# pyannote/pyannote-audio

Measured on AMD Instinct MI355X. Metric: audio-hours/sec (real-time factor) for speaker-diarization-3.1 pipeline, higher is better.
Workload: dtype f32

## Files before the change

pyannote-audio_amd/csrc/emb_winograd4.hip:

```cpp
#include <stdlib.h>

#include <type_traits>

#include "common.h"
#include "emb_winograd_geom.h"
#include "emb_winograd4_geom.h"

namespace pa {

typedef float f32x2 __attribute__((ext_vector_type(2)));
typedef __attribute__((address_space(3))) void* lds4_ptr_t;

typedef const volatile f32x2 __attribute__((address_space(3))) * w4_lds_f32x2_ptr;
__device__ __forceinline__ f32x2 w4_lds_read64(const unsigned char* p) { return *(w4_lds_f32x2_ptr)p; }

__device__ __forceinline__ void wino4_barrier() {
  asm volatile("s_waitcnt lgkmcnt(0)" ::: "memory");
  __builtin_amdgcn_s_barrier();
  asm volatile("" ::: "memory");
}

struct W4Const {
  f32x2 p4, m4, m5, p2, m2, m1;
};
__device__ __forceinline__ f32x2 w4fma(f32x2 a, f32x2 b, f32x2 c) { return __builtin_elementwise_fma(a, b, c); }
__device__ __forceinline__ void wino4_bt(const f32x2 (&x)[6], f32x2 (&y)[6], const W4Const& k) {
  const f32x2 a = w4fma(x[2], k.m4, x[4]);
  const f32x2 b = w4fma(x[1], k.m4, x[3]);
  const f32x2 c = w4fma(x[2], k.m1, x[4]);
  const f32x2 d = w4fma(x[1], k.m1, x[3]);
  y[0] = w4fma(x[0], k.p4, w4fma(x[2], k.m5, x[4]));
  y[1] = a + b;
  y[2] = w4fma(b, k.m1, a);
  y[3] = w4fma(d, k.p2, c);
  y[4] = w4fma(d, k.m2, c);
  y[5] = w4fma(x[1], k.p4, w4fma(x[3], k.m5, x[5]));
}

struct W4Const4 {
  f32x4 m1, p2, p4, p8, m2, m8;
};
__device__ __forceinline__ f32x4 w4fma4(f32x4 a, f32x4 b, f32x4 c) { return __builtin_elementwise_fma(a, b, c); }
__device__ __forceinline__ void wino4_at(const f32x4 m0, const f32x4 m1, const f32x4 m2, const f32x4 m3,
                                         const f32x4 m4, const f32x4 m5, f32x4 (&y)[4], const W4Const4& k) {
  const f32x4 s1 = m1 + m2, d1 = w4fma4(m2, k.m1, m1), s2 = m3 + m4, d2 = w4fma4(m4, k.m1, m3);
  y[0] = m0 + s1 + s2;
  y[1] = w4fma4(d2, k.p2, d1);
  y[2] = w4fma4(s2, k.p4, s1);
  y[3] = w4fma4(d2, k.p8, d1) + m5;
}

#define W4_MFMA_A(acc, a, b) asm volatile("v_mfma_f32_16x16x4_f32 %0, %1, %2, %0" : "+a"(acc) : "v"(a), "v"(b))
#define W4_MFMA_A_ZERO(acc, a, b) asm volatile("v_mfma_f32_16x16x4_f32 %0, %1, %2, 0" : "=a"(acc) : "v"(a), "v"(b))
#define W4_MFMA_V(acc, a, b) asm volatile("v_mfma_f32_16x16x4_f32 %0, %1, %2, %0" : "+v"(acc) : "v"(a), "v"(b))
#define W4_MFMA_V_ZERO(acc, a, b) asm volatile("v_mfma_f32_16x16x4_f32 %0, %1, %2, 0" : "=v"(acc) : "v"(a), "v"(b))

__device__ __forceinline__ float w4_opaque(float v) {
  asm volatile("" : "+s"(v));
  return v;
}

struct Wino4Stage {
  __amdgpu_buffer_rsrc_t xsrd, usrd;
  int keep, usoff;
  unsigned char* pbuf;
  unsigned char* ubuf;
};
struct Wino4Ctx {
  const float* xp;
  int xnum;
  int keep, usoff;
};
__device__ __forceinline__ Wino4Ctx wino4_ctx(const float* __restrict__ X, int H, int W, int CIN, const Wino4Unit& u,
                                              int n0, int x0_last) {
  using G = Wino4Geom;
  const long img = (long)H * W * CIN;
  const long org = ((long)(u.y0 - 1) * W + (u.x0 - 1)) * CIN;
  Wino4Ctx c;
  c.xp = X + (long)u.b * img + org;
  c.xnum = (int)((img - org) * 4);
  c.keep = wino4_patch_keep(u, x0_last);
  c.usoff = (n0 / W_BN) * (CIN / G::CB) * G::USLAB_BYTES;
  return c;
}
__device__ __forceinline__ Wino4Stage wino4_stage(const Wino4Ctx& c, const float* __restrict__ U, int COUT, int CIN,
                                                  int s, unsigned char* pbuf, unsigned char* ubuf) {
  using G = Wino4Geom;
  Wino4Stage st;
  st.xsrd = __builtin_amdgcn_make_buffer_rsrc(const_cast<float*>(c.xp + s * G::CB), 0, c.xnum - s * G::CB * 4,
                                              0x00020000);
  st.usrd = __builtin_amdgcn_make_buffer_rsrc(const_cast<float*>(U), 0, 36 * COUT * CIN * 4, 0x00020000);
  st.keep = c.keep;
  st.usoff = c.usoff + s * G::USLAB_BYTES;
  st.pbuf = pbuf;
  st.ubuf = ubuf;
  return st;
}

#ifndef PA_W4_STAMP
#define PA_W4_STAMP 0
#endif
#ifndef PA_W4_DEFER_STORES
#define PA_W4_DEFER_STORES 1
#endif
#ifndef PA_W4_STORE_AUX
#define PA_W4_STORE_AUX 2
#endif
#ifndef PA_W4_RES_AUX
#define PA_W4_RES_AUX 0
#endif
#ifndef PA_W4_STORES_IN_FLIGHT
#define PA_W4_STORES_IN_FLIGHT 1
#endif
#ifndef PA_W4_LATE_BARRIER
#define PA_W4_LATE_BARRIER 1
#endif
#if PA_W4_STAMP
__device__ unsigned long long g_w4_stamps[8 * 4 * 64 * 10];
#define W4_STAMP(p) st_[p] = __builtin_amdgcn_s_memtime()
#define W4_STAMP_FLUSH()                                                                      \
  do {                                                                                        \
    if (blockIdx.x < 8 && st_iter < 64 && lane == 0) {                                         \
      _Pragma("unroll") for (int p_ = 0; p_ < 10; ++p_)                                        \
          g_w4_stamps[((blockIdx.x * 4 + slw) * 64 + st_iter) * 10 + p_] = st_[p_];            \
    }                                                                                         \
    ++st_iter;                                                                                \
  } while (0)
#else
#define W4_STAMP(p)
#define W4_STAMP_FLUSH()
#endif

constexpr int W4_AGPR_POINTS = 32;
constexpr int W4_U_PIECES = Wino4Geom::UINSTR / 4;
static_assert(W4_U_PIECES == 9 && Wino4Geom::UINSTR % 4 == 0, "36 U pieces of 1 KB per stage, 4 waves");
constexpr int W4_TILE_OUT = 16;
constexpr int W4_TAIL_WAIT = 2 * W4_TILE_OUT;
#define W4_STR2(x) #x
#define W4_STR(x) W4_STR2(x)
#define W4_U_PIECES_LIT 9
#define W4_TAIL_WAIT_LIT 32
static_assert(W4_U_PIECES == W4_U_PIECES_LIT && W4_TAIL_WAIT == W4_TAIL_WAIT_LIT, "the literals of the s_waitcnt strings");

template <int PIN>
struct Wino4Lanes {
  int a[PIN];
};
template <int PIN>
__device__ __forceinline__ void wino4_piece(const int I, const Wino4Stage& st, const Wino4Lanes<PIN>& pl, int lane,
                                            int slw) {
  if (I < PIN) {
    const int off = pl.a[I < PIN ? I : 0] & st.keep;
    __builtin_amdgcn_raw_ptr_buffer_load_lds(st.xsrd, (lds4_ptr_t)(st.pbuf + 1024 * I), 16, off, 0, 0, 0);
  } else {
    const int k = slw + 4 * (I - PIN);
    __builtin_amdgcn_raw_ptr_buffer_load_lds(st.usrd, (lds4_ptr_t)(st.ubuf + 1024 * k), 16, lane * 16,
                                             st.usoff + 1024 * k, 0, 0);
  }
}
struct Wino4Dma {
  unsigned patch_lds;
  unsigned u_lds;
  int usoff;
};
__device__ __forceinline__ unsigned w4_lds_addr(const void* p) {
  return (unsigned)(size_t)(lds4_ptr_t)const_cast<void*>(p);
}
template <int I, int PIN>
__device__ __forceinline__ void wino4_piece_asm(const Wino4Stage& st, const Wino4Dma& d, const int (&plm)[PIN],
                                                int lane16) {
  if constexpr (I < PIN) {
    asm volatile("s_add_u32 m0, %0, %1\n\ts_nop 0\n\tbuffer_load_dwordx4 %2, %3, 0 offen lds"
                 :: "s"(d.patch_lds), "i"(1024 * I), "v"(plm[I]), "s"(st.xsrd)
                 : "memory");
  } else {
    int tmp;
    asm volatile("s_add_u32 m0, %1, %2\n\ts_add_u32 %0, %3, %2\n\tbuffer_load_dwordx4 %4, %5, %0 offen lds"
                 : "=&s"(tmp)
                 : "s"(d.u_lds), "i"(4096 * (I - PIN)), "s"(d.usoff), "v"(lane16), "s"(st.usrd)
                 : "memory");
  }
}
template <int PIN>
__device__ __forceinline__ void wino4_piece_asm_n(const int piece, const Wino4Stage& st, const Wino4Dma& d,
                                                  const int (&plm)[PIN], int lane16) {
  switch (piece) {
#define W4_CASE(I) case I: if constexpr (I < PIN + W4_U_PIECES) wino4_piece_asm<I, PIN>(st, d, plm, lane16); break;
    W4_CASE(0) W4_CASE(1) W4_CASE(2) W4_CASE(3) W4_CASE(4) W4_CASE(5) W4_CASE(6) W4_CASE(7) W4_CASE(8) W4_CASE(9)
    W4_CASE(10) W4_CASE(11) W4_CASE(12) W4_CASE(13) W4_CASE(14) W4_CASE(15) W4_CASE(16) W4_CASE(17) W4_CASE(18)
    W4_CASE(19) W4_CASE(20) W4_CASE(21) W4_CASE(22) W4_CASE(23) W4_CASE(24) W4_CASE(25) W4_CASE(26)
#undef W4_CASE
    default: break;
  }
}
template <int PIN>
__device__ __forceinline__ void wino4_issue_all(const Wino4Stage& st, const Wino4Lanes<PIN>& pl, int lane, int slw) {
#pragma unroll
  for (int i = 0; i < PIN + W4_U_PIECES; ++i) wino4_piece<PIN>(i, st, pl, lane, slw);
}

struct Wino4LinUnit {
  int b0;
  Wino4LinTile tc;
};
__device__ __forceinline__ Wino4LinUnit wino4_lin_unit(int u, int tcols, int trows, int total_tiles, int H, int W,
                                                       int CIN, int lane, int (&off)[Wino4LinGeom::PINSTR]) {
  Wino4LinUnit o;
  o.b0 = __builtin_amdgcn_readfirstlane(wino4_lin_b0(u, tcols, trows, total_tiles));
  o.tc = wino4_lin_tile(16 * u + (lane & 15), tcols, trows, total_tiles, o.b0);
  const Wino4LinTile td = wino4_lin_tile(16 * u + ((lane >> 1) & 15), tcols, trows, total_tiles, o.b0);
#pragma unroll
  for (int i = 0; i < Wino4LinGeom::PINSTR; ++i) off[i] = wino4_lin_patch_lane(i, td, H, W, CIN, lane);
  return o;
}
__device__ __forceinline__ Wino4LinUnit wino4_run_unit(int u, int tcols, int trows, int total_tiles, int H, int W,
                                                       int CIN, int nimg, int lane, int (&off)[Wino4RunGeom::PINSTR],
                                                       int* slot) {
  Wino4LinUnit o;
  int b0;
  const Wino4Runs R = wino4_runs(u, tcols, trows, &b0);
  o.b0 = __builtin_amdgcn_readfirstlane(b0);
  const int t = lane & 15;
  o.tc = wino4_run_tile(R, t, u, total_tiles);
  *slot = t + wino4_run_of_tile(R, t);
  wino4_run_patch_lanes(off, R, H, W, CIN, nimg - o.b0, lane);
  return o;
}
__device__ __forceinline__ Wino4Ctx wino4_lin_ctx(const float* __restrict__ X, int H, int W, int CIN, int nimg, int b0,
                                                  int n0) {
  using G = Wino4LinGeom;
  const long img = (long)H * W * CIN;
  const long long rest = (long long)(nimg - b0) * img * 4;
  Wino4Ctx c;
  c.xp = X + (long)b0 * img;
  c.xnum = (int)(rest > 0x7fffffffLL ? 0x7fffffffLL : rest);
  c.keep = -1;
  c.usoff = (n0 / W_BN) * (CIN / G::CB) * G::USLAB_BYTES;
  return c;
}

template <bool HAS_R, int MODE>
__global__ __launch_bounds__(256, 1) void k_conv3x3_wino4(
    const float* __restrict__ X, int H, int W, int CIN, const float* __restrict__ U,
    const float* __restrict__ shift, const float* __restrict__ R, float* __restrict__ Y, int COUT, int relu,
    int cgroups, int trows, int num_units, int num_groups, int n_tiles, int total_work, int nimg, int xranges,
    int* __restrict__ counters) {
  constexpr bool LATE = PA_W4_LATE_BARRIER && MODE == 0;
  constexpr bool LIN = MODE != 0;
  constexpr bool RUN = MODE == 2;
  using G = std::conditional_t<MODE == 0, Wino4Geom, std::conditional_t<MODE == 1, Wino4LinGeom, Wino4RunGeom>>;
  constexpr int PIN = G::PINSTR;
  constexpr int W4_PIECES = PIN + W4_U_PIECES;
  static_assert(W4_PIECES <= 27, "wino4_piece_asm_n spells out 27 cases");
  static_assert(2 * W4_TILE_OUT * (HAS_R ? 2 : 1) >= W4_TAIL_WAIT, "a tile's first-stage wait counts epilogue operations");
  extern __shared__ __attribute__((aligned(16))) unsigned char smem4[];
  const int tid = threadIdx.x, lane = tid & 63;
  const int t = lane & 15, g = lane >> 4;
  const int slw = __builtin_amdgcn_readfirstlane(tid >> 6);
  unsigned char* my_patch = smem4 + slw * G::PATCH_BYTES;
  unsigned char* ubufs = smem4 + 4 * G::PATCH_BYTES;
  int* mail = reinterpret_cast<int*>(smem4 + G::LDS_BYTES);

  const TileQueue tq{counters, (int)(blockIdx.x & 7), total_work >> 3};
  if (tid == 0) mail[0] = tq_resolve(tq, tq_claim_own(tq));
  __syncthreads();
  int q = mail[0];
  if (q < 0) {
    if (tid == 0) tq_done(tq, gridDim.x);
    return;
  }
  const int x0_last = LIN ? 0 : (cgroups - 1) * Wino4Geom::TW;
  Wino4Lanes<PIN> pl;
  Wino4Lanes<PIN> npl;
  if constexpr (!LIN) wino4_patch_lanes(pl.a, W, CIN, lane, x0_last);
#define W4_PATCH_K(i, j) (MODE == 1 ? wino4_lin_patch_k(i, j) : (MODE == 2 ? wino4_run_patch_k(i, j) : wino4_patch_k(i, j)))
  int pbase0 = MODE == 1 ? wino4_lin_patch_base(t, g) : wino4_patch_base(t, g, 0);
  int pbase1 = MODE == 1 ? pbase0 : wino4_patch_base(t, g, 1);
  int nxt_slot = 0;
  const int last_unit = LIN ? ((num_units + 15) >> 4) - 1 : 0;
  const int ubase = wino4_u_base(t, g);
  const int lane16 = lane * 16;
  W4Const kc;
  {
    const float p4 = w4_opaque(4.f), m4 = w4_opaque(-4.f), m5 = w4_opaque(-5.f), p2 = w4_opaque(2.f),
                m2 = w4_opaque(-2.f), m1 = w4_opaque(-1.f);
    kc.p4 = f32x2{p4, p4}; kc.m4 = f32x2{m4, m4}; kc.m5 = f32x2{m5, m5};
    kc.p2 = f32x2{p2, p2}; kc.m2 = f32x2{m2, m2}; kc.m1 = f32x2{m1, m1};
  }
  const int nstages = CIN / G::CB;

  Wino4Work wk = wino4_decode(q, n_tiles, num_groups, xranges);
  Wino4Unit cur = Wino4Unit{0, 0, 0, 0}, nxt = cur;
  Wino4LinUnit lcur = Wino4LinUnit{0, Wino4LinTile{0, 0, 0, 0}}, lnxt = lcur;
  int cur_n0 = wk.n0, nxt_n0 = wk.n0;
  Wino4Ctx cctx;
  if constexpr (RUN) {
    const int uu = wk.unit0 + slw;
    int slot;
    lcur = wino4_run_unit(uu < last_unit ? uu : last_unit, cgroups, trows, num_units, H, W, CIN, nimg, lane, pl.a, &slot);
    lcur.tc.valid &= wk.valid & (uu <= last_unit);
    pbase0 = wino4_run_patch_base(slot, g, 0);
    pbase1 = wino4_run_patch_base(slot, g, 1);
    cctx = wino4_lin_ctx(X, H, W, CIN, nimg, lcur.b0, cur_n0);
  } else if constexpr (LIN) {
    lcur = wino4_lin_unit(wk.unit0 + slw, cgroups, trows, num_units, H, W, CIN, lane, pl.a);
    lcur.tc.valid &= wk.valid;
    cctx = wino4_lin_ctx(X, H, W, CIN, nimg, lcur.b0, cur_n0);
  } else {
    cur = wino4_unit(wk.unit0 + slw, cgroups, trows, num_units);
    cur.valid &= wk.valid;
    cctx = wino4_ctx(X, H, W, CIN, cur, cur_n0, x0_last);
  }
  nxt = cur;
  lnxt = lcur;
  Wino4Ctx nctx = cctx;
  int buf = 0;
  wino4_issue_all<PIN>(wino4_stage(cctx, U, COUT, CIN, 0, my_patch, ubufs), pl, lane, slw);
  int claim = 0;
  if (tid == 0) claim = tq_claim_own(tq);
  int nq = -1;
  bool first_tile = true;
  f32x4 acca[W4_AGPR_POINTS][2];
  f32x4 accv[36 - W4_AGPR_POINTS][2];

#if PA_W4_STAMP
  unsigned long long st_[10] = {0, 0, 0, 0, 0, 0, 0, 0, 0, 0};
  int st_iter = 0;
#endif
  while (true) {
    for (int s = 0; s < nstages; ++s) {
      W4_STAMP(0);
      if constexpr (LATE) {
      if (s == 0) {
        if (PA_W4_STORES_IN_FLIGHT && !first_tile) asm volatile("s_waitcnt vmcnt(" W4_STR(W4_TAIL_WAIT_LIT) ")" ::: "memory");
        else asm volatile("s_waitcnt vmcnt(0)" ::: "memory");
      } else {
        asm volatile("s_waitcnt vmcnt(" W4_STR(W4_U_PIECES_LIT) ")" ::: "memory");
      }
      } else {
        asm volatile("s_waitcnt vmcnt(0)" ::: "memory");
      }
      W4_STAMP(1);
      if (s == nstages - 1 && tid == 0) mail[0] = tq_resolve(tq, claim);
      f32x2 x_first[6];
      asm volatile("s_waitcnt lgkmcnt(0)" ::: "memory");
#pragma unroll
      for (int i = 0; i < 6; ++i)
        x_first[i] = w4_lds_read64(my_patch + pbase0 + W4_PATCH_K(i, 0));
      unsigned char* umine = ubufs + buf * G::USLAB_BYTES;
      unsigned char* uother = ubufs + (buf ^ 1) * G::USLAB_BYTES;
      bool stage_next = true;
      Wino4Stage nst;
      auto stage_barrier = [&]() {
        if constexpr (LATE) asm volatile("s_waitcnt vmcnt(0)" ::: "memory");
        __builtin_amdgcn_s_barrier();
        asm volatile("" ::: "memory");
        W4_STAMP(2);
        if (s + 1 < nstages) {
          nst = wino4_stage(cctx, U, COUT, CIN, s + 1, my_patch, uother);
        } else {
          nq = mail[0];
          stage_next = nq >= 0;
          wk = wino4_decode(stage_next ? nq : 0, n_tiles, num_groups, xranges);
          nxt_n0 = wk.n0;
          if constexpr (LIN) {
            const int uu = wk.unit0 + slw;
            if constexpr (RUN) {
              lnxt = wino4_run_unit(uu < last_unit ? uu : last_unit, cgroups, trows, num_units, H, W, CIN, nimg, lane,
                                    npl.a, &nxt_slot);
              lnxt.tc.valid &= wk.valid & (uu <= last_unit);
            } else {
              lnxt = wino4_lin_unit(uu, cgroups, trows, num_units, H, W, CIN, lane, npl.a);
              lnxt.tc.valid &= wk.valid;
            }
            nctx = wino4_lin_ctx(X, H, W, CIN, nimg, lnxt.b0, nxt_n0);
          } else {
            nxt = wino4_unit(wk.unit0 + slw, cgroups, trows, num_units);
            nxt.valid &= wk.valid;
            nctx = wino4_ctx(X, H, W, CIN, nxt, nxt_n0, x0_last);
          }
          nst = wino4_stage(nctx, U, COUT, CIN, 0, my_patch, uother);
        }
      };
      if constexpr (!LATE) stage_barrier();
      f32x2 v[6][6];
      f32x2 uf_first[2][2];
      {
        const unsigned char* pb0 = my_patch + pbase0;
        const unsigned char* pb1 = my_patch + pbase1;
        f32x2 tt[6][6];
        f32x2 x[2][6];
#define W4_RD(i, j) w4_lds_read64(((j) >> 2 ? pb1 : pb0) + W4_PATCH_K(i, j))
#pragma unroll
        for (int i = 0; i < 6; ++i) x[0][i] = x_first[i];
#pragma unroll
        for (int j = 0; j < 6; ++j) {
          if (j + 1 < 6) {
#pragma unroll
            for (int i = 0; i < 6; ++i) x[(j + 1) & 1][i] = W4_RD(i, j + 1);
          }
          __builtin_amdgcn_sched_barrier(0);
          f32x2 y[6];
          wino4_bt(x[j & 1], y, kc);
#pragma unroll
          for (int i = 0; i < 6; ++i) tt[i][j] = y[i];
          __builtin_amdgcn_sched_barrier(0);
        }
#pragma unroll
        for (int i = 0; i < 6; ++i) {
          if (i == 5) {
            if constexpr (LATE) {
              stage_barrier();
              __builtin_amdgcn_sched_barrier(0);
            }
#pragma unroll
            for (int e = 0; e < 2; ++e)
#pragma unroll
              for (int cg = 0; cg < 2; ++cg) uf_first[e][cg] = w4_lds_read64(umine + ubase + wino4_u_k(e, cg));
            __builtin_amdgcn_sched_barrier(0);
          }
          wino4_bt(tt[i], v[i], kc);
          __builtin_amdgcn_sched_barrier(0);
        }
      }
#if PA_W4_STAMP
      asm volatile("s_nop 0" ::"v"(v[5][5]), "v"(v[0][0]));
#endif
      W4_STAMP(3);
      int plm[PIN];
      if constexpr (LIN) {
#pragma unroll
        for (int i = 0; i < PIN; ++i) plm[i] = s + 1 < nstages ? pl.a[i] : npl.a[i];
      } else {
#pragma unroll
        for (int i = 0; i < PIN; ++i) plm[i] = pl.a[i] & nst.keep;
      }
      const Wino4Dma dma{w4_lds_addr(my_patch), w4_lds_addr(uother) + 1024u * slw, nst.usoff + 1024 * slw};
      auto mfma_run = [&](auto first_stage) {
        constexpr bool FIRST = decltype(first_stage)::value;
        const unsigned char* ub = umine + ubase;
        f32x2 uf[2][2][2];
#pragma unroll
        for (int e = 0; e < 2; ++e)
#pragma unroll
          for (int cg = 0; cg < 2; ++cg) {
            uf[0][e][cg] = uf_first[e][cg];
          }
        __builtin_amdgcn_sched_barrier(0);
#pragma unroll
        for (int xp = 0; xp < 36; xp += 2) {
          const int par = (xp >> 1) & 1;
#pragma unroll
          for (int m = 0; m < 8; ++m) {
            const int ks = m >> 2, e = (m >> 1) & 1, cg = m & 1;
            const int xi = xp + e;
            const f32x2 bv = v[xi / 6][xi % 6];
            const float a = ks ? uf[par][e][cg].y : uf[par][e][cg].x, b = ks ? bv.y : bv.x;
            if (xi < W4_AGPR_POINTS) {
              if (ks == 0 && FIRST) W4_MFMA_A_ZERO(acca[xi < W4_AGPR_POINTS ? xi : 0][cg], a, b);
              else W4_MFMA_A(acca[xi < W4_AGPR_POINTS ? xi : 0][cg], a, b);
            } else {
              if (ks == 0 && FIRST) W4_MFMA_V_ZERO(accv[xi >= W4_AGPR_POINTS ? xi - W4_AGPR_POINTS : 0][cg], a, b);
              else W4_MFMA_V(accv[xi >= W4_AGPR_POINTS ? xi - W4_AGPR_POINTS : 0][cg], a, b);
            }
            __builtin_amdgcn_sched_barrier(0);
            if ((m == 0 || m == 2) && xp + 2 < 36) {
              const int en = m >> 1;
#pragma unroll
              for (int c2 = 0; c2 < 2; ++c2)
                uf[par ^ 1][en][c2] = w4_lds_read64(ub + wino4_u_k(xp + 2 + en, c2));
              __builtin_amdgcn_sched_barrier(0);
            }
            if ((m == 4 || m == 6) && stage_next) {
              const int piece = xp + ((m - 4) >> 1);
              if (piece < W4_PIECES) wino4_piece_asm_n<PIN>(piece, nst, dma, plm, lane16);
              __builtin_amdgcn_sched_barrier(0);
            }
          }
        }
      };
      if (s == 0) mfma_run(std::true_type{});
      else mfma_run(std::false_type{});
      W4_STAMP(4);
      buf ^= 1;
      if (s + 1 < nstages) {
        W4_STAMP(5);
        W4_STAMP_FLUSH();
      }
    }
    if (tid == 0 && nq >= 0) claim = tq_claim_own(tq);
    first_tile = false;
    asm volatile("s_nop 15\n\ts_nop 15" ::: "memory");
    {
      W4Const4 k4;
      {
        const float m1 = w4_opaque(-1.f), p2 = w4_opaque(2.f), p4 = w4_opaque(4.f), p8 = w4_opaque(8.f),
                    m2 = w4_opaque(-2.f), m8 = w4_opaque(-8.f);
        k4.m1 = f32x4{m1, m1, m1, m1}; k4.p2 = f32x4{p2, p2, p2, p2};
        k4.p4 = f32x4{p4, p4, p4, p4}; k4.p8 = f32x4{p8, p8, p8, p8};
        k4.m2 = f32x4{m2, m2, m2, m2}; k4.m8 = f32x4{m8, m8, m8, m8};
      }
      const long oimg = (long)H * W * COUT;
      const int ob = LIN ? lcur.b0 : cur.b;
      const long long orest = (long long)(LIN ? nimg - ob : 1) * oimg * 4;
      const int onum = (int)(orest > 0x7fffffffLL ? 0x7fffffffLL : orest);
      const __amdgpu_buffer_rsrc_t ysrd = __builtin_amdgcn_make_buffer_rsrc(Y + (long)ob * oimg, 0, onum, 0x00020000);
      const __amdgpu_buffer_rsrc_t rsrd = __builtin_amdgcn_make_buffer_rsrc(
          const_cast<float*>(HAS_R ? R + (long)ob * oimg : Y), 0, onum, 0x00020000);
      constexpr int OOB = (int)0x80000000;
      const int xl = LIN ? lcur.tc.x : cur.x0 + 4 * t;
      const int yl = LIN ? lcur.tc.b * H + lcur.tc.y : cur.y0;
      const int rows_ok = LIN ? H - lcur.tc.y : 4;
      const int tile_ok = LIN ? lcur.tc.valid : cur.valid;
      const int obase = ((yl * W + xl) * COUT + cur_n0 + 4 * g) * 4;
      const int srow = W * COUT * 4, spix = COUT * 4;
      int offq[4];
#pragma unroll
      for (int qq = 0; qq < 4; ++qq) offq[qq] = (tile_ok && xl + qq < W) ? obase + qq * spix : OOB;
      auto ooff = [&](const int p, const int qq, const int cg) {
        if constexpr (LIN) return (offq[qq] == OOB || p >= rows_ok) ? OOB : offq[qq] + p * srow + 64 * cg;
        else return offq[qq] == OOB ? OOB : offq[qq] + p * srow + 64 * cg;
      };
      const float lo = relu ? 0.f : -__builtin_inff();
      const f32x4 lo4 = {lo, lo, lo, lo};
#define W4_ACC(xi) ((xi) < W4_AGPR_POINTS ? acca[(xi) < W4_AGPR_POINTS ? (xi) : 0][cg] \
                                          : accv[(xi) >= W4_AGPR_POINTS ? (xi)-W4_AGPR_POINTS : 0][cg])
      constexpr bool DEFER = PA_W4_DEFER_STORES == 2 || (PA_W4_DEFER_STORES == 1 && !HAS_R);
      f32x4 held[4][4];
      auto store_held = [&](const int k) {
        __builtin_amdgcn_raw_buffer_store_b128(__builtin_bit_cast(u32x4, held[k >> 2][k & 3]), ysrd,
                                               ooff(k >> 2, k & 3, 0), 0, PA_W4_STORE_AUX);
      };
#pragma unroll
      for (int cg = 0; cg < 2; ++cg) {
        f32x4 sh;
        {
          const float* sp = shift + cur_n0 + 16 * cg;
          float s16[16];
#pragma unroll
          for (int i = 0; i < 16; ++i) s16[i] = sp[i];
#pragma unroll
          for (int r = 0; r < 4; ++r)
            sh[r] = g == 0 ? s16[r] : (g == 1 ? s16[4 + r] : (g == 2 ? s16[8 + r] : s16[12 + r]));
        }
        f32x4 rv[4][4];
        if (HAS_R) {
#pragma unroll
          for (int p = 0; p < 2; ++p)
#pragma unroll
            for (int qq = 0; qq < 4; ++qq)
              rv[p][qq] = __builtin_bit_cast(
                  f32x4, __builtin_amdgcn_raw_buffer_load_b128(rsrd, ooff(p, qq, cg), 0, PA_W4_RES_AUX));
        }
        __builtin_amdgcn_sched_barrier(0);
        f32x4 o[4][4];
#pragma unroll
        for (int b = 0; b < 6; ++b) {
#pragma unroll
          for (int a6 = 0; a6 < 6; ++a6) {
            const int xi = 6 * a6 + b;
            if (xi < W4_AGPR_POINTS) asm volatile("" : "+a"(acca[xi < W4_AGPR_POINTS ? xi : 0][cg]));
          }
          f32x4 y[4];
          wino4_at(W4_ACC(0 + b), W4_ACC(6 + b), W4_ACC(12 + b), W4_ACC(18 + b), W4_ACC(24 + b), W4_ACC(30 + b), y,
                   k4);
#pragma unroll
          for (int p = 0; p < 4; ++p) {
            if (b == 0) {
              o[p][0] = y[p];
            } else if (b == 1) {
              o[p][0] = o[p][0] + y[p];
              o[p][1] = y[p];
              o[p][2] = y[p];
              o[p][3] = y[p];
            } else if (b == 2) {
              o[p][0] = o[p][0] + y[p];
              o[p][1] = w4fma4(y[p], k4.m1, o[p][1]);
              o[p][2] = o[p][2] + y[p];
              o[p][3] = w4fma4(y[p], k4.m1, o[p][3]);
            } else if (b == 3) {
              o[p][0] = o[p][0] + y[p];
              o[p][1] = w4fma4(y[p], k4.p2, o[p][1]);
              o[p][2] = w4fma4(y[p], k4.p4, o[p][2]);
              o[p][3] = w4fma4(y[p], k4.p8, o[p][3]);
            } else if (b == 4) {
              o[p][0] = o[p][0] + y[p];
              o[p][1] = w4fma4(y[p], k4.m2, o[p][1]);
              o[p][2] = w4fma4(y[p], k4.p4, o[p][2]);
              o[p][3] = w4fma4(y[p], k4.m8, o[p][3]);
            } else {
              o[p][3] = o[p][3] + y[p];
            }
          }
          if (b & 1) __builtin_amdgcn_sched_barrier(0);
          if (DEFER && cg == 1) {
            constexpr int first[7] = {0, 3, 6, 9, 12, 14, 16};
            __builtin_amdgcn_sched_barrier(0);
#pragma unroll
            for (int k = first[b]; k < first[b + 1]; ++k) store_held(k);
            __builtin_amdgcn_sched_barrier(0);
          }
          if (HAS_R && b == 3) {
#pragma unroll
            for (int p = 2; p < 4; ++p)
#pragma unroll
              for (int qq = 0; qq < 4; ++qq)
                rv[p][qq] = __builtin_bit_cast(
                    f32x4, __builtin_amdgcn_raw_buffer_load_b128(rsrd, ooff(p, qq, cg), 0, PA_W4_RES_AUX));
            __builtin_amdgcn_sched_barrier(0);
          }
        }
#if PA_W4_STAMP
        asm volatile("s_nop 0" ::"v"(o[3][3]), "v"(o[0][0]));
        st_[6 + 2 * cg] = __builtin_amdgcn_s_memtime();
#endif
#pragma unroll
        for (int p = 0; p < 4; ++p)
#pragma unroll
          for (int qq = 0; qq < 4; ++qq) {
            o[p][qq] = o[p][qq] + sh;
            if (HAS_R) o[p][qq] = o[p][qq] + rv[p][qq];
            o[p][qq] = __builtin_elementwise_max(o[p][qq], lo4);
          }
        __builtin_amdgcn_sched_barrier(0);
        if (DEFER && cg == 0) {
#pragma unroll
          for (int p = 0; p < 4; ++p)
#pragma unroll
            for (int qq = 0; qq < 4; ++qq) held[p][qq] = o[p][qq];
        } else {
#pragma unroll
          for (int p = 0; p < 4; ++p)
#pragma unroll
            for (int qq = 0; qq < 4; ++qq)
              __builtin_amdgcn_raw_buffer_store_b128(__builtin_bit_cast(u32x4, o[p][qq]), ysrd, ooff(p, qq, cg), 0,
                                                     PA_W4_STORE_AUX);
        }
        __builtin_amdgcn_sched_barrier(0);
#if PA_W4_STAMP
        st_[7 + 2 * cg] = __builtin_amdgcn_s_memtime();
#endif
      }
#undef W4_ACC
    }
    W4_STAMP(5);
    W4_STAMP_FLUSH();
    if (nq < 0) break;
    cur = nxt;
    if constexpr (LIN) {
      lcur = lnxt;
      pl = npl;
      if constexpr (RUN) {
        pbase0 = wino4_run_patch_base(nxt_slot, g, 0);
        pbase1 = wino4_run_patch_base(nxt_slot, g, 1);
      }
    }
    cur_n0 = nxt_n0;
    cctx = nctx;
  }
  if (tid == 0) tq_done(tq, gridDim.x);
}

static int wino4_unit_mode(int B, int H, int W, int rows) {
  if (rows != H) return 0;
  const long tcols = cdiv(W, 4), trows = cdiv(H, 4);
  static const char* e = getenv("PA_WINO4_LINEAR");
  if (e != nullptr) {
    const int m = atoi(e);
    return m == 2 && tcols < 5 ? 1 : m;
  }
  const long lin_units = cdiv((long)B * trows * tcols, 16), row_units = (long)B * trows * cdiv(W, 64);
  if (tcols >= 5 && lin_units * 118 <= row_units * 100) return 2;
  return lin_units * 120 <= row_units * 100 ? 1 : 0;
}

int xcd_ranges_wanted(bool by_default) {
  static const char* e = getenv("PA_XCD_RANGES");
  return e != nullptr ? (atoi(e) != 0) : (by_default ? 1 : 0);
}

template <bool HAS_R, int MODE>
static int launch_wino4(const float* X, int B, int H, int W, int CIN, const float* U, const float* shift,
                        const float* R, float* Y, int COUT, int relu, int rows, hipStream_t st) {
  constexpr bool LIN = MODE != 0;
  using G = std::conditional_t<MODE == 0, Wino4Geom, std::conditional_t<MODE == 1, Wino4LinGeom, Wino4RunGeom>>;
  const int cgroups = LIN ? cdiv(W, 4) : cdiv(W, Wino4Geom::TW), trows = cdiv(rows, 4);
  const size_t lds = (size_t)G::LDS_BYTES + 16;
  auto kernel = k_conv3x3_wino4<HAS_R, MODE>;
  constexpr int MAXDEV = 16;
  static int cus_of[MAXDEV] = {0};
  int dev = 0;
  (void)hipGetDevice(&dev);
  if (dev < 0 || dev >= MAXDEV) dev = 0;
  if (!cus_of[dev]) {
    (void)hipFuncSetAttribute((const void*)kernel, hipFuncAttributeMaxDynamicSharedMemorySize, (int)lds);
    int cus = 256;
    (void)hipDeviceGetAttribute(&cus, hipDeviceAttributeMultiprocessorCount, dev);
    cus_of[dev] = cus;
  }
  const int n_tiles = COUT / W_BN;
  const long total_tiles = (long)cgroups * trows * B;
  const long num_units = LIN ? (total_tiles + 15) / 16 : (long)cgroups * trows * B;
  const long num_groups = (num_units + 3) / 4;
  const long total = ((num_groups + 7) / 8) * 8 * n_tiles;
  const int resident = cus_of[dev] & ~7;
  const int grid = (int)(total < resident ? total : resident);
  int* counters = tile_counters();
  if (counters == nullptr) {
    set_error("pa_conv3x3_wino4: cannot allocate the tile counters");
    return 2;
  }
  hipLaunchKernelGGL(kernel, dim3(grid), dim3(256), lds, st, X, H, W, CIN, U, shift, R, Y, COUT, relu, cgroups, trows,
                     (int)(LIN ? total_tiles : num_units), (int)num_groups, n_tiles, (int)total, B,
                     xcd_ranges_wanted(n_tiles < 8), counters);
  return 0;
}

}

extern "C" {

#if PA_W4_STAMP
int pa_wino4_read_stamps(unsigned long long* host) {
  (void)hipDeviceSynchronize();
  return hipMemcpyFromSymbol(host, HIP_SYMBOL(pa::g_w4_stamps), sizeof(unsigned long long) * 8 * 4 * 64 * 10) ==
                 hipSuccess
             ? 0
             : 1;
}
#endif

int pa_conv3x3_wino4_rows(const float* X, int B, int H, int W, int cin, const float* U, const float* shift,
                          const float* R, float* Y, int cout, int relu, int rows, void* stream);

int pa_conv3x3_wino4(const float* X, int B, int H, int W, int cin, const float* U, const float* shift,
                     const float* R, float* Y, int cout, int relu, void* stream) {
  return pa_conv3x3_wino4_rows(X, B, H, W, cin, U, shift, R, Y, cout, relu, H, stream);
}

int pa_conv3x3_wino4_rows(const float* X, int B, int H, int W, int cin, const float* U, const float* shift,
                          const float* R, float* Y, int cout, int relu, int rows, void* stream) {
  if (B <= 0 || rows <= 0) return 0;
  PA_REQUIRE(rows == H || (rows < H && rows % 4 == 0), "pa_conv3x3_wino4_rows: rows must be H or a multiple of 4 below it");
  PA_REQUIRE(cin % 8 == 0 && cin >= 32 && cout % pa::W_BN == 0,
             "pa_conv3x3_wino4: cin %% 8 == 0, cin >= 32 and cout %% 32 == 0 required");
  PA_REQUIRE((long)H * W * (cin > cout ? cin : cout) * 4 < (1L << 28),
             "pa_conv3x3_wino4: one image must be smaller than 256 MB");
  pa::ProfScope prof("k_conv3x3_wino4", stream, 2.0 * 9 * cin * cout * (double)B * rows * W,
                     4.0 * ((double)B * rows * W * cin + (double)B * rows * W * cout * (R ? 2 : 1) + 9.0 * cin * cout));
  hipStream_t st = (hipStream_t)stream;
  int rc;
  const int mode = pa::wino4_unit_mode(B, H, W, rows);
  if (mode != 0) {
    const long per = (long)pa::cdiv(H, 4) * pa::cdiv(W, 4);
    const long span = (15 / per + 2) * (long)H * W * (cin > cout ? cin : cout) * 4;
    PA_REQUIRE(span < (1L << 31), "pa_conv3x3_wino4: the images a 16-tile unit can touch must stay below 2 GB");
  }
  if (mode == 2)
    rc = R != nullptr ? pa::launch_wino4<true, 2>(X, B, H, W, cin, U, shift, R, Y, cout, relu, rows, st)
                      : pa::launch_wino4<false, 2>(X, B, H, W, cin, U, shift, R, Y, cout, relu, rows, st);
  else if (mode == 1)
    rc = R != nullptr ? pa::launch_wino4<true, 1>(X, B, H, W, cin, U, shift, R, Y, cout, relu, rows, st)
                      : pa::launch_wino4<false, 1>(X, B, H, W, cin, U, shift, R, Y, cout, relu, rows, st);
  else
    rc = R != nullptr ? pa::launch_wino4<true, 0>(X, B, H, W, cin, U, shift, R, Y, cout, relu, rows, st)
                      : pa::launch_wino4<false, 0>(X, B, H, W, cin, U, shift, R, Y, cout, relu, rows, st);
  if (rc != 0) return rc;
  PA_CHECK_LAUNCH("pa_conv3x3_wino4");
  return 0;
}

}
```

Before: 1.305.

## Pair adjacent lanes in Winograd epilogue to write contiguous 128-byte output runs

In the no-residual path of the Winograd F(4,3) conv epilogue, both channel groups are now computed first and then exchanged between adjacent lanes with DPP cndmask, so each lane pair stores 32 contiguous channels of one pixel instead of two strided 64-byte halves. The first group's outputs are parked in AGPRs in linear modes to limit VGPR pressure, and all stores are issued together at the end instead of interleaved with the second group's output transform. The goal is better write coalescing, at the cost of extra cross-lane moves, AGPR traffic and losing the overlap of stores with compute. An unpaired variant is kept for testing.

Result: no change. 1.311 (median of 6 runs) (+0.5%).

```diff
diff --git a/pyannote-audio_amd/csrc/emb_winograd4.hip b/pyannote-audio_amd/csrc/emb_winograd4.hip
--- a/pyannote-audio_amd/csrc/emb_winograd4.hip
+++ b/pyannote-audio_amd/csrc/emb_winograd4.hip
@@ -100,9 +100,6 @@
 #ifndef PA_W4_STAMP
 #define PA_W4_STAMP 0
 #endif
-#ifndef PA_W4_DEFER_STORES
-#define PA_W4_DEFER_STORES 1
-#endif
 #ifndef PA_W4_STORE_AUX
 #define PA_W4_STORE_AUX 2
 #endif
@@ -239,7 +236,7 @@
   return c;
 }
 
-template <bool HAS_R, int MODE>
+template <bool HAS_R, int MODE, bool PAIR = true>
 __global__ __launch_bounds__(256, 1) void k_conv3x3_wino4(
     const float* __restrict__ X, int H, int W, int CIN, const float* __restrict__ U,
     const float* __restrict__ shift, const float* __restrict__ R, float* __restrict__ Y, int COUT, int relu,
@@ -517,129 +514,290 @@
       int offq[4];
 #pragma unroll
       for (int qq = 0; qq < 4; ++qq) offq[qq] = (tile_ok && xl + qq < W) ? obase + qq * spix : OOB;
-      auto ooff = [&](const int p, const int qq, const int cg) {
-        if constexpr (LIN) return (offq[qq] == OOB || p >= rows_ok) ? OOB : offq[qq] + p * srow + 64 * cg;
-        else return offq[qq] == OOB ? OOB : offq[qq] + p * srow + 64 * cg;
-      };
       const float lo = relu ? 0.f : -__builtin_inff();
       const f32x4 lo4 = {lo, lo, lo, lo};
 #define W4_ACC(xi) ((xi) < W4_AGPR_POINTS ? acca[(xi) < W4_AGPR_POINTS ? (xi) : 0][cg] \
                                           : accv[(xi) >= W4_AGPR_POINTS ? (xi)-W4_AGPR_POINTS : 0][cg])
-      constexpr bool DEFER = PA_W4_DEFER_STORES == 2 || (PA_W4_DEFER_STORES == 1 && !HAS_R);
-      f32x4 held[4][4];
-      auto store_held = [&](const int k) {
-        __builtin_amdgcn_raw_buffer_store_b128(__builtin_bit_cast(u32x4, held[k >> 2][k & 3]), ysrd,
-                                               ooff(k >> 2, k & 3, 0), 0, PA_W4_STORE_AUX);
-      };
-#pragma unroll
-      for (int cg = 0; cg < 2; ++cg) {
-        f32x4 sh;
+      if constexpr (!HAS_R) {
+        const bool odd = (lane & 1) != 0;
+        auto swap1 = [](const int v) { return __builtin_amdgcn_mov_dpp(v, 0xB1, 0xF, 0xF, true); };
+        int offs[2][4], rows_s[2];
+        auto slot_offsets = [&]() {
+    #pragma unroll
+          for (int qq = 0; qq < 4; ++qq) {
+            const int mine = offq[qq] == OOB ? OOB : offq[qq] + (PAIR ? (odd ? 64 : 0) : 0);
+            if constexpr (PAIR) {
+              const int theirs = swap1(offq[qq]);
+              const int other = theirs == OOB ? OOB : theirs + (odd ? 64 : 0);
+              offs[0][qq] = odd ? other : mine;
+              offs[1][qq] = odd ? mine : other;
+            } else {
+              offs[0][qq] = mine;
+              offs[1][qq] = mine == OOB ? OOB : mine + 64;
+            }
+          }
+          if constexpr (PAIR && LIN) {
+            const int theirs = swap1(rows_ok);
+            rows_s[0] = odd ? theirs : rows_ok;
+            rows_s[1] = odd ? rows_ok : theirs;
+          } else {
+            rows_s[0] = rows_s[1] = rows_ok;
+          }
+        };
+        auto soff = [&](const int p, const int qq, const int sl) {
+          const int o = offs[sl][qq];
+          if constexpr (LIN) return (o == OOB || p >= rows_s[sl]) ? OOB : o + p * srow;
+          else return o == OOB ? OOB : o + p * srow;
+        };
+        f32x4 shs[2];
         {
-          const float* sp = shift + cur_n0 + 16 * cg;
-          float s16[16];
-#pragma unroll
-          for (int i = 0; i < 16; ++i) s16[i] = sp[i];
-#pragma unroll
-          for (int r = 0; r < 4; ++r)
-            sh[r] = g == 0 ? s16[r] : (g == 1 ? s16[4 + r] : (g == 2 ? s16[8 + r] : s16[12 + r]));
+          f32x4 sh[2];
+#pragma unroll
+          for (int cg = 0; cg < 2; ++cg) {
+            const float* sp = shift + cur_n0 + 16 * cg;
+            float s16[16];
+#pragma unroll
+            for (int i = 0; i < 16; ++i) s16[i] = sp[i];
+#pragma unroll
+            for (int r = 0; r < 4; ++r)
+              sh[cg][r] = g == 0 ? s16[r] : (g == 1 ? s16[4 + r] : (g == 2 ? s16[8 + r] : s16[12 + r]));
+          }
+          shs[0] = PAIR ? (odd ? sh[1] : sh[0]) : sh[0];
+          shs[1] = PAIR ? shs[0] : sh[1];
         }
-        f32x4 rv[4][4];
-        if (HAS_R) {
-#pragma unroll
-          for (int p = 0; p < 2; ++p)
-#pragma unroll
-            for (int qq = 0; qq < 4; ++qq)
-              rv[p][qq] = __builtin_bit_cast(
-                  f32x4, __builtin_amdgcn_raw_buffer_load_b128(rsrd, ooff(p, qq, cg), 0, PA_W4_RES_AUX));
+        auto store_row = [&](const int p, f32x4 (&w0)[4][4], f32x4 (&w1)[4][4]) {
+#pragma unroll
+          for (int qq = 0; qq < 4; ++qq) {
+            __builtin_amdgcn_raw_buffer_store_b128(__builtin_bit_cast(u32x4, w0[p][qq]), ysrd, soff(p, qq, 0), 0,
+                                                   PA_W4_STORE_AUX);
+            __builtin_amdgcn_raw_buffer_store_b128(__builtin_bit_cast(u32x4, w1[p][qq]), ysrd, soff(p, qq, 1), 0,
+                                                   PA_W4_STORE_AUX);
+          }
+        };
+        f32x4 held[4][4];
+        constexpr bool PARK = LIN;
+        float parked[4][4][4];
+        f32x4 o[4][4];
+#pragma unroll
+        for (int cg = 0; cg < 2; ++cg) {
+          __builtin_amdgcn_sched_barrier(0);
+#pragma unroll
+          for (int b = 0; b < 6; ++b) {
+#pragma unroll
+            for (int a6 = 0; a6 < 6; ++a6) {
+              const int xi = 6 * a6 + b;
+              if (xi < W4_AGPR_POINTS) asm volatile("" : "+a"(acca[xi < W4_AGPR_POINTS ? xi : 0][cg]));
+            }
+            f32x4 y[4];
+            wino4_at(W4_ACC(0 + b), W4_ACC(6 + b), W4_ACC(12 + b), W4_ACC(18 + b), W4_ACC(24 + b), W4_ACC(30 + b), y,
+                     k4);
+#pragma unroll
+            for (int p = 0; p < 4; ++p) {
+              if (b == 0) {
+                o[p][0] = y[p];
+              } else if (b == 1) {
+                o[p][0] = o[p][0] + y[p];
+                o[p][1] = y[p];
+                o[p][2] = y[p];
+                o[p][3] = y[p];
+              } else if (b == 2) {
+                o[p][0] = o[p][0] + y[p];
+                o[p][1] = w4fma4(y[p], k4.m1, o[p][1]);
+                o[p][2] = o[p][2] + y[p];
+                o[p][3] = w4fma4(y[p], k4.m1, o[p][3]);
+              } else if (b == 3) {
+                o[p][0] = o[p][0] + y[p];
+                o[p][1] = w4fma4(y[p], k4.p2, o[p][1]);
+                o[p][2] = w4fma4(y[p], k4.p4, o[p][2]);
+                o[p][3] = w4fma4(y[p], k4.p8, o[p][3]);
+              } else if (b == 4) {
+                o[p][0] = o[p][0] + y[p];
+                o[p][1] = w4fma4(y[p], k4.m2, o[p][1]);
+                o[p][2] = w4fma4(y[p], k4.p4, o[p][2]);
+                o[p][3] = w4fma4(y[p], k4.m8, o[p][3]);
+              } else {
+                o[p][3] = o[p][3] + y[p];
+              }
+            }
+            if (b & 1) __builtin_amdgcn_sched_barrier(0);
+          }
+#if PA_W4_STAMP
+          asm volatile("s_nop 0" ::"v"(o[3][3]), "v"(o[0][0]));
+          st_[6 + 2 * cg] = __builtin_amdgcn_s_memtime();
+          if (cg == 0) st_[7] = st_[6];
+#endif
+          if (cg == 0) {
+#pragma unroll
+            for (int p = 0; p < 4; ++p)
+#pragma unroll
+              for (int qq = 0; qq < 4; ++qq) {
+                if constexpr (PARK) {
+#pragma unroll
+                  for (int r = 0; r < 4; ++r)
+                    asm volatile("v_accvgpr_write_b32 %0, %1" : "=a"(parked[p][qq][r]) : "v"(o[p][qq][r]));
+                } else {
+                  held[p][qq] = o[p][qq];
+                }
+              }
+          }
+        }
+        slot_offsets();
+        __builtin_amdgcn_sched_barrier(0);
+        const unsigned long long even_mask = 0x5555555555555555ull;
+        auto finish = [&](const f32x4 v, const int sl) { return __builtin_elementwise_max(v + shs[sl], lo4); };
+#pragma unroll
+        for (int p = 0; p < 4; ++p) {
+#pragma unroll
+          for (int qq = 0; qq < 4; ++qq) {
+            f32x4 w0, w1;
+            if constexpr (PARK) {
+#pragma unroll
+              for (int r = 0; r < 4; ++r)
+                asm volatile("v_accvgpr_read_b32 %0, %1" : "=v"(held[p][qq][r]) : "a"(parked[p][qq][r]));
+            }
+            if constexpr (PAIR) {
+              float t0, t1, t2, t3;
+              float b0 = o[p][qq][0], b1 = o[p][qq][1], b2 = o[p][qq][2], b3 = o[p][qq][3];
+#define W4_XDPP " quad_perm:[1,0,3,2] row_mask:0xf bank_mask:0xf\n\t"
+              asm volatile("s_nop 1\n\ts_mov_b64 vcc, %12\n\t"
+                           "v_cndmask_b32_dpp %0, %4, %8, vcc" W4_XDPP
+                           "v_cndmask_b32_dpp %1, %5, %9, vcc" W4_XDPP
+                           "v_cndmask_b32_dpp %2, %6, %10, vcc" W4_XDPP
+                           "v_cndmask_b32_dpp %3, %7, %11, vcc" W4_XDPP
+                           "s_not_b64 vcc, vcc\n\t"
+                           "v_cndmask_b32_dpp %4, %8, %4, vcc" W4_XDPP
+                           "v_cndmask_b32_dpp %5, %9, %5, vcc" W4_XDPP
+                           "v_cndmask_b32_dpp %6, %10, %6, vcc" W4_XDPP
+                           "v_cndmask_b32_dpp %7, %11, %7, vcc" W4_XDPP
+                           : "=&v"(t0), "=&v"(t1), "=&v"(t2), "=&v"(t3), "+v"(b0), "+v"(b1), "+v"(b2), "+v"(b3)
+                           : "v"(held[p][qq][0]), "v"(held[p][qq][1]), "v"(held[p][qq][2]), "v"(held[p][qq][3]),
+                             "s"(even_mask)
+                           : "vcc", "scc");
+#undef W4_XDPP
+              w0 = f32x4{t0, t1, t2, t3};
+              w1 = f32x4{b0, b1, b2, b3};
+            } else {
+              w0 = held[p][qq];
+              w1 = o[p][qq];
+            }
+            held[p][qq] = finish(w0, 0);
+            o[p][qq] = finish(w1, 1);
+          }
+          __builtin_amdgcn_sched_barrier(0);
+        }
+#pragma unroll
+        for (int p = 0; p < 4; ++p) store_row(p, held, o);
+        if constexpr (PARK) {
+#pragma unroll
+          for (int xi = 0; xi < W4_AGPR_POINTS; ++xi)
+#pragma unroll
+            for (int cg = 0; cg < 2; ++cg) asm volatile("" : "=a"(acca[xi][cg]));
         }
         __builtin_amdgcn_sched_barrier(0);
-        f32x4 o[4][4];
-#pragma unroll
-        for (int b = 0; b < 6; ++b) {
-#pragma unroll
-          for (int a6 = 0; a6 < 6; ++a6) {
-            const int xi = 6 * a6 + b;
-            if (xi < W4_AGPR_POINTS) asm volatile("" : "+a"(acca[xi < W4_AGPR_POINTS ? xi : 0][cg]));
-          }
-          f32x4 y[4];
-          wino4_at(W4_ACC(0 + b), W4_ACC(6 + b), W4_ACC(12 + b), W4_ACC(18 + b), W4_ACC(24 + b), W4_ACC(30 + b), y,
-                   k4);
-#pragma unroll
-          for (int p = 0; p < 4; ++p) {
-            if (b == 0) {
-              o[p][0] = y[p];
-            } else if (b == 1) {
-              o[p][0] = o[p][0] + y[p];
-              o[p][1] = y[p];
-              o[p][2] = y[p];
-              o[p][3] = y[p];
-            } else if (b == 2) {
-              o[p][0] = o[p][0] + y[p];
-              o[p][1] = w4fma4(y[p], k4.m1, o[p][1]);
-              o[p][2] = o[p][2] + y[p];
-              o[p][3] = w4fma4(y[p], k4.m1, o[p][3]);
-            } else if (b == 3) {
-              o[p][0] = o[p][0] + y[p];
-              o[p][1] = w4fma4(y[p], k4.p2, o[p][1]);
-              o[p][2] = w4fma4(y[p], k4.p4, o[p][2]);
-              o[p][3] = w4fma4(y[p], k4.p8, o[p][3]);
-            } else if (b == 4) {
-              o[p][0] = o[p][0] + y[p];
-              o[p][1] = w4fma4(y[p], k4.m2, o[p][1]);
-              o[p][2] = w4fma4(y[p], k4.p4, o[p][2]);
-              o[p][3] = w4fma4(y[p], k4.m8, o[p][3]);
-            } else {
-              o[p][3] = o[p][3] + y[p];
-            }
-          }
-          if (b & 1) __builtin_amdgcn_sched_barrier(0);
-          if (DEFER && cg == 1) {
-            constexpr int first[7] = {0, 3, 6, 9, 12, 14, 16};
-            __builtin_amdgcn_sched_barrier(0);
-#pragma unroll
-            for (int k = first[b]; k < first[b + 1]; ++k) store_held(k);
-            __builtin_amdgcn_sched_barrier(0);
-          }
-          if (HAS_R && b == 3) {
-#pragma unroll
-            for (int p = 2; p < 4; ++p)
+#if PA_W4_STAMP
+        st_[9] = __builtin_amdgcn_s_memtime();
+#endif
+      } else {
+        auto ooff = [&](const int p, const int qq, const int cg) {
+          if constexpr (LIN) return (offq[qq] == OOB || p >= rows_ok) ? OOB : offq[qq] + p * srow + 64 * cg;
+          else return offq[qq] == OOB ? OOB : offq[qq] + p * srow + 64 * cg;
+        };
+#pragma unroll
+        for (int cg = 0; cg < 2; ++cg) {
+          f32x4 sh;
+          {
+            const float* sp = shift + cur_n0 + 16 * cg;
+            float s16[16];
+#pragma unroll
+            for (int i = 0; i < 16; ++i) s16[i] = sp[i];
+#pragma unroll
+            for (int r = 0; r < 4; ++r)
+              sh[r] = g == 0 ? s16[r] : (g == 1 ? s16[4 + r] : (g == 2 ? s16[8 + r] : s16[12 + r]));
+          }
+          f32x4 rv[4][4];
+          {
+#pragma unroll
+            for (int p = 0; p < 2; ++p)
 #pragma unroll
               for (int qq = 0; qq < 4; ++qq)
                 rv[p][qq] = __builtin_bit_cast(
                     f32x4, __builtin_amdgcn_raw_buffer_load_b128(rsrd, ooff(p, qq, cg), 0, PA_W4_RES_AUX));
-            __builtin_amdgcn_sched_barrier(0);
-          }
-        }
+          }
+          __builtin_amdgcn_sched_barrier(0);
+          f32x4 o[4][4];
+#pragma unroll
+          for (int b = 0; b < 6; ++b) {
+#pragma unroll
+            for (int a6 = 0; a6 < 6; ++a6) {
+              const int xi = 6 * a6 + b;
+              if (xi < W4_AGPR_POINTS) asm volatile("" : "+a"(acca[xi < W4_AGPR_POINTS ? xi : 0][cg]));
+            }
+            f32x4 y[4];
+            wino4_at(W4_ACC(0 + b), W4_ACC(6 + b), W4_ACC(12 + b), W4_ACC(18 + b), W4_ACC(24 + b), W4_ACC(30 + b), y,
+                     k4);
+#pragma unroll
+            for (int p = 0; p < 4; ++p) {
+              if (b == 0) {
+                o[p][0] = y[p];
+              } else if (b == 1) {
+                o[p][0] = o[p][0] + y[p];
+                o[p][1] = y[p];
+                o[p][2] = y[p];
+                o[p][3] = y[p];
+              } else if (b == 2) {
+                o[p][0] = o[p][0] + y[p];
+                o[p][1] = w4fma4(y[p], k4.m1, o[p][1]);
+                o[p][2] = o[p][2] + y[p];
+                o[p][3] = w4fma4(y[p], k4.m1, o[p][3]);
+              } else if (b == 3) {
+                o[p][0] = o[p][0] + y[p];
+                o[p][1] = w4fma4(y[p], k4.p2, o[p][1]);
+                o[p][2] = w4fma4(y[p], k4.p4, o[p][2]);
+                o[p][3] = w4fma4(y[p], k4.p8, o[p][3]);
+              } else if (b == 4) {
+                o[p][0] = o[p][0] + y[p];
+                o[p][1] = w4fma4(y[p], k4.m2, o[p][1]);
+                o[p][2] = w4fma4(y[p], k4.p4, o[p][2]);
+                o[p][3] = w4fma4(y[p], k4.m8, o[p][3]);
+              } else {
+                o[p][3] = o[p][3] + y[p];
+              }
+            }
+            if (b & 1) __builtin_amdgcn_sched_barrier(0);
+            if (b == 3) {
+#pragma unroll
+              for (int p = 2; p < 4; ++p)
+#pragma unroll
+                for (int qq = 0; qq < 4; ++qq)
+                  rv[p][qq] = __builtin_bit_cast(
+                      f32x4, __builtin_amdgcn_raw_buffer_load_b128(rsrd, ooff(p, qq, cg), 0, PA_W4_RES_AUX));
+              __builtin_amdgcn_sched_barrier(0);
+            }
+          }
 #if PA_W4_STAMP
-        asm volatile("s_nop 0" ::"v"(o[3][3]), "v"(o[0][0]));
-        st_[6 + 2 * cg] = __builtin_amdgcn_s_memtime();
-#endif
-#pragma unroll
-        for (int p = 0; p < 4; ++p)
-#pragma unroll
-          for (int qq = 0; qq < 4; ++qq) {
-            o[p][qq] = o[p][qq] + sh;
-            if (HAS_R) o[p][qq] = o[p][qq] + rv[p][qq];
-            o[p][qq] = __builtin_elementwise_max(o[p][qq], lo4);
-          }
-        __builtin_amdgcn_sched_barrier(0);
-        if (DEFER && cg == 0) {
+          asm volatile("s_nop 0" ::"v"(o[3][3]), "v"(o[0][0]));
+          st_[6 + 2 * cg] = __builtin_amdgcn_s_memtime();
+#endif
 #pragma unroll
           for (int p = 0; p < 4; ++p)
 #pragma unroll
-            for (int qq = 0; qq < 4; ++qq) held[p][qq] = o[p][qq];
-        } else {
+            for (int qq = 0; qq < 4; ++qq) {
+              o[p][qq] = o[p][qq] + sh;
+              o[p][qq] = o[p][qq] + rv[p][qq];
+              o[p][qq] = __builtin_elementwise_max(o[p][qq], lo4);
+            }
+          __builtin_amdgcn_sched_barrier(0);
 #pragma unroll
           for (int p = 0; p < 4; ++p)
 #pragma unroll
             for (int qq = 0; qq < 4; ++qq)
               __builtin_amdgcn_raw_buffer_store_b128(__builtin_bit_cast(u32x4, o[p][qq]), ysrd, ooff(p, qq, cg), 0,
                                                      PA_W4_STORE_AUX);
+          __builtin_amdgcn_sched_barrier(0);
+#if PA_W4_STAMP
+          st_[7 + 2 * cg] = __builtin_amdgcn_s_memtime();
+#endif
         }
-        __builtin_amdgcn_sched_barrier(0);
-#if PA_W4_STAMP
-        st_[7 + 2 * cg] = __builtin_amdgcn_s_memtime();
-#endif
       }
 #undef W4_ACC
     }
@@ -679,14 +837,14 @@
   return e != nullptr ? (atoi(e) != 0) : (by_default ? 1 : 0);
 }
 
-template <bool HAS_R, int MODE>
+template <bool HAS_R, int MODE, bool PAIR = true>
 static int launch_wino4(const float* X, int B, int H, int W, int CIN, const float* U, const float* shift,
                         const float* R, float* Y, int COUT, int relu, int rows, hipStream_t st) {
   constexpr bool LIN = MODE != 0;
   using G = std::conditional_t<MODE == 0, Wino4Geom, std::conditional_t<MODE == 1, Wino4LinGeom, Wino4RunGeom>>;
   const int cgroups = LIN ? cdiv(W, 4) : cdiv(W, Wino4Geom::TW), trows = cdiv(rows, 4);
   const size_t lds = (size_t)G::LDS_BYTES + 16;
-  auto kernel = k_conv3x3_wino4<HAS_R, MODE>;
+  auto kernel = k_conv3x3_wino4<HAS_R, MODE, PAIR>;
   constexpr int MAXDEV = 16;
   static int cus_of[MAXDEV] = {0};
   int dev = 0;
@@ -738,8 +896,19 @@
   return pa_conv3x3_wino4_rows(X, B, H, W, cin, U, shift, R, Y, cout, relu, H, stream);
 }
 
+static int conv3x3_wino4_rows(const float* X, int B, int H, int W, int cin, const float* U, const float* shift,
+                              const float* R, float* Y, int cout, int relu, int rows, bool pair, void* stream);
 int pa_conv3x3_wino4_rows(const float* X, int B, int H, int W, int cin, const float* U, const float* shift,
                           const float* R, float* Y, int cout, int relu, int rows, void* stream) {
+  return conv3x3_wino4_rows(X, B, H, W, cin, U, shift, R, Y, cout, relu, rows, true, stream);
+}
+int patest_conv3x3_wino4_unpaired(const float* X, int B, int H, int W, int cin, const float* U, const float* shift,
+                              const float* R, float* Y, int cout, int relu, void* stream) {
+  return conv3x3_wino4_rows(X, B, H, W, cin, U, shift, R, Y, cout, relu, H, false, stream);
+}
+
+static int conv3x3_wino4_rows(const float* X, int B, int H, int W, int cin, const float* U, const float* shift,
+                              const float* R, float* Y, int cout, int relu, int rows, bool pair, void* stream) {
   if (B <= 0 || rows <= 0) return 0;
   PA_REQUIRE(rows == H || (rows < H && rows % 4 == 0), "pa_conv3x3_wino4_rows: rows must be H or a multiple of 4 below it");
   PA_REQUIRE(cin % 8 == 0 && cin >= 32 && cout % pa::W_BN == 0,
@@ -758,13 +927,16 @@
   }
   if (mode == 2)
     rc = R != nullptr ? pa::launch_wino4<true, 2>(X, B, H, W, cin, U, shift, R, Y, cout, relu, rows, st)
-                      : pa::launch_wino4<false, 2>(X, B, H, W, cin, U, shift, R, Y, cout, relu, rows, st);
+                      : (pair ? pa::launch_wino4<false, 2>(X, B, H, W, cin, U, shift, R, Y, cout, relu, rows, st)
+                              : pa::launch_wino4<false, 2, false>(X, B, H, W, cin, U, shift, R, Y, cout, relu, rows, st));
   else if (mode == 1)
     rc = R != nullptr ? pa::launch_wino4<true, 1>(X, B, H, W, cin, U, shift, R, Y, cout, relu, rows, st)
-                      : pa::launch_wino4<false, 1>(X, B, H, W, cin, U, shift, R, Y, cout, relu, rows, st);
+                      : (pair ? pa::launch_wino4<false, 1>(X, B, H, W, cin, U, shift, R, Y, cout, relu, rows, st)
+                              : pa::launch_wino4<false, 1, false>(X, B, H, W, cin, U, shift, R, Y, cout, relu, rows, st));
   else
     rc = R != nullptr ? pa::launch_wino4<true, 0>(X, B, H, W, cin, U, shift, R, Y, cout, relu, rows, st)
-                      : pa::launch_wino4<false, 0>(X, B, H, W, cin, U, shift, R, Y, cout, relu, rows, st);
+                      : (pair ? pa::launch_wino4<false, 0>(X, B, H, W, cin, U, shift, R, Y, cout, relu, rows, st)
+                              : pa::launch_wino4<false, 0, false>(X, B, H, W, cin, U, shift, R, Y, cout, relu, rows, st));
   if (rc != 0) return rc;
   PA_CHECK_LAUNCH("pa_conv3x3_wino4");
   return 0;
```
